# fzaiser/genfer

Measured on AMD Instinct MI355X. Metric: TaylorPoly mul f64 GMAC/s, higher is better.
Workload: dtype f64

## Files before the change

genfer_amd/csrc/gft_api.hip:

```cpp
#include <hip/hip_runtime.h>
#include <dlfcn.h>
#include <rccl/rccl.h>

#include <algorithm>
#include <chrono>
#include <atomic>
#include <cmath>
#include <cstdio>
#include <cstring>
#include <deque>
#include <exception>
#include <functional>
#include <initializer_list>
#include <map>
#include <memory>
#include <tuple>
#include <stdexcept>
#include <string>
#include <vector>

#include "../../include/gftaylor.h"
#include "gft_kernels.hpp"
#include "gft_small_alloc.hpp"
#include "gft_host.hpp"
// ... 159 lines not shown
    size_t peak_total = 0;
    unsigned* d_flag = nullptr;
    double* d_scratch = nullptr;
    unsigned* d_wit = nullptr;
    double* h_pinned = nullptr;
    double* h_mail = nullptr;
    double* d_mail = nullptr;
    unsigned long long mail_seq = 0;
    hipEvent_t events[64] = {};
    static constexpr int IO_EVENTS = 16;
    hipEvent_t io_events[IO_EVENTS] = {};
    int io_next = 0;
    int series_force = 0;
    int series_last = 0;
    int conv_mode = 0;
    static constexpr int pairs_first = 1;
    double pairs_first_max = 1.0e7, pairs_first_max_rank2 = 2.0e8;
    double tiled_min_macs = 2.0e5;
    double tiled_min_override = -1;
    static constexpr double recur_tiled_min_macs = 1.0e300;
    size_t stats[8] = {0, 0, 0, 0, 0, 0, 0, 0};
    size_t stats_ex[4] = {0, 0, 0, 0};
    bool defer = true;
    size_t horner_loop_max = (size_t)1 << 40;
    static constexpr bool fuse_horner = true;
    bool div_wavefront = true;
    bool exp_right = true;
    size_t shallow_max_terms = 256;
    size_t stats_shallow[2] = {0, 0};
    unsigned nf_epoch = 0;
    int conv_variant = -1;
    void* conv_ws = nullptr;
    size_t conv_ws_bytes = 0;
    void ensure_conv_ws(size_t need) {
        if (need <= conv_ws_bytes) return;
        size_t want = std::max<size_t>(std::max(need, std::min<size_t>(2 * conv_ws_bytes, (size_t)1 << 32)), (size_t)8 << 20);
        if (conv_ws) HIP_OK(hipFree(conv_ws));
        conv_ws = nullptr;
        conv_ws_bytes = 0;
        if (hipMalloc(&conv_ws, want) != hipSuccess) {
            (void)hipGetLastError();
            want = need;
            HIP_OK(hipMalloc(&conv_ws, want));
        }
        conv_ws_bytes = want;
    }
    unsigned* next_nf_epoch() {
        if (++nf_epoch == 0) {
            HIP_OK(hipMemsetD32Async((hipDeviceptr_t)(d_flag + 2), 0, 1, stream));
            nf_epoch = 1;
        }
        return d_flag + 2;
    }
    static constexpr size_t HOST_MAX_ELEMS_DEFAULT = 2048;
    static constexpr double HOST_MAX_MACS_DEFAULT = 65536;
    size_t host_max_elems = HOST_MAX_ELEMS_DEFAULT;
    double host_max_macs = HOST_MAX_MACS_DEFAULT;
    std::map<size_t, std::vector<void*>> host_blocks;
};
Runtime& R = *new Runtime;

static size_t size_class(size_t bytes) {
    if (bytes < 256) return 256;
    if (bytes <= (1u << 20)) {
        size_t c = 256;
        while (c < bytes) c <<= 1;
        return c;
    }
    const size_t g = 2u << 20;
// ... 1020 lines not shown
        HIP_OK(hipEventSynchronize(R.events[b]));
        float ms = 0;
        HIP_OK(hipEventElapsedTime(&ms, R.events[a], R.events[b]));
        return ms;
    } catch (const std::exception& e) {
        g_err = e.what();
        return -1.0f;
    }
}
int gft_set_option(const char* name, double value) {
    std::string n = name ? name : "";
    if (n == "horner_loop_max") R.horner_loop_max = value < 0 ? 0 : (size_t)value;
    else if (n == "div_wavefront") R.div_wavefront = value != 0;
    else if (n == "exp_right") R.exp_right = value != 0;
    else if (n == "recur_overlap") R.recur_overlap = value != 0;
    else if (n == "defer") R.defer = value != 0;
    else if (n == "lazy_observe") R.lazy_observe = value != 0;
    else if (n == "batch_dag") R.batch_dag = value != 0;
    else if (n == "lazy_horner") R.lazy_horner = value != 0;
    else if (n == "nz_proofs") R.nz_proofs = value != 0;
    else if (n == "lazy_sum") R.lazy_sum = value != 0;
    else if (n == "async_launch") lq_configure(R.device, value != 0);
    else if (n == "trace_lq_report") lq_report();
    else if (n == "shallow_max_terms") R.shallow_max_terms = value < 0 ? 256 : (size_t)value;
    else if (n == "debug_fail_next_launch") g_fail_next_launch.store(value != 0 ? 1 : 0);
    else if (n == "tiled_min_macs") R.tiled_min_macs = value;
    else if (n == "conv_rb_min_macs") staged_set_rb_min_macs(value);
    else if (n == "conv_rb_pairs") staged_set_rb_pairs(value);
    else if (n == "conv_rb_pairs_cap") staged_set_rb_pairs_cap(value);
    else if (n == "conv_rb_pairs_lanes") staged_set_rb_pairs_lanes(value);
    else if (n == "shallow_pair_min") shallow_set_pair_min(value == -1.0 ? 4096.0 : value);
    else if (n == "tiled_tile") tiled_set_lane_tile((int)value);
    else if (n == "tiled_peel") tiled_set_peel((int)value);
    else if (n == "host_max_elems") R.host_max_elems = value < 0 ? Runtime::HOST_MAX_ELEMS_DEFAULT : (size_t)value;
    else if (n == "host_max_macs") R.host_max_macs = value < 0 ? Runtime::HOST_MAX_MACS_DEFAULT : value;
    else if (n == "series_form") R.series_force = (value == 1 || value == 2) ? (int)value : 0;
    else if (n == "dist_min_macs") dist_set_min_macs(value);
    else if (n == "dist_event_slot") dist_set_event_slot(value);
    else return -1;
    return 0;
}
int gft_set_conv_variant(int v) {
    R.conv_variant = v;
    return 0;
}
int gft_set_conv_mode(int mode) {
    if (mode < 0 || mode > 3) return -1;
    R.conv_mode = mode;
    return 0;
}

int gft_conv_raw(const double* x, const size_t* xshape, const double* y, const size_t* yshape, double* res,
                 const size_t* rshape, size_t ndim, size_t slab_lo, size_t slab_hi, int accumulate) {
    return guard_int([&] {
        typedef Ops<EF64> O;
        O::HV xv{const_cast<double*>(x), 0, dims(xshape, ndim)};
        O::HV yv{const_cast<double*>(y), 0, dims(yshape, ndim)};
        O::HV zv{res, 0, dims(rshape, ndim)};
        for (size_t i = 0; i < ndim; ++i)
            if (xshape[i] > rshape[i] || yshape[i] > rshape[i] || xshape[i] == 0 || yshape[i] == 0)
                throw Error("conv_raw: operand shapes must be non-empty and not exceed the result shape");
        if (ndim > 0 && (slab_lo > slab_hi || slab_hi > rshape[0])) throw Error("conv_raw: bad slab range");
        O::conv(xv, yv, zv, slab_lo, slab_hi, accumulate != 0, false, 0, 0, 0);
        launch_drain();
        return 0;
    });
// ... 564 lines not shown
```

genfer_amd/csrc/gft_conv_tiled.hip:

```cpp
#include <algorithm>
#include <cstdlib>
#include <cstring>
#include <map>
#include <vector>

#include "gft_kernels.hpp"

namespace gft {

namespace {

struct TileSeg {
    unsigned u, a, b;
    unsigned step_begin, step_end;
    int dest;
};

struct RedTile {
    unsigned u, a, b;
    unsigned first, count;
    unsigned slot0;
};

struct TiledArgs {
    unsigned xU, x0, x1, xI;
    unsigned yU, y0, y1, yI;
    unsigned zU, z0, z1, zI;
    unsigned nx8, ny8;
    unsigned nxc, nyc, nb;
    unsigned P1;
    unsigned tsh;
    unsigned slab_axis;
    unsigned slab_lo, slab_hi;
    int accumulate;
    unsigned xcd_remap;
    unsigned cut;
    unsigned lim1;
    size_t zsU, zs0, zs1, zoff;
    const double* xp;
    const double* yp;
    double* z;
    double* ws;
    const TileSeg* segs;
    const unsigned* wg_begin;
    const RedTile* red;
    const unsigned* red_slots;
    const unsigned* guard;
    unsigned guard_epoch;
    unsigned char blk1[8], blk2[8];
};

typedef const double __attribute__((address_space(4))) * cptr_t;

#ifndef GFT_TILED_DEFAULT_VARIANT
#define GFT_TILED_DEFAULT_VARIANT 7
#endif
#ifndef GFT_TILED_PEEL_DEFAULT
#define GFT_TILED_PEEL_DEFAULT -1
#endif
constexpr unsigned PEEL_MIN_EXTENT = 112, PEEL_MIN_INNER = 64;

__device__ inline void loadx(double (&dst)[8], cptr_t p) {
#pragma unroll
    for (int i = 0; i < 8; ++i) dst[i] = p[i];
}

__device__ inline void load8(double (&dst)[8], const double* p) {
#pragma unroll
    for (int i = 0; i < 8; ++i) dst[i] = p[i];
}

__device__ inline void load8_b128(double (&dst)[8], const double* p) {
    const double2* q = reinterpret_cast<const double2*>(__builtin_assume_aligned(p, 16));
#pragma unroll
    for (int i = 0; i < 4; ++i) {
        double2 v = q[i];
        dst[2 * i] = v.x;
        dst[2 * i + 1] = v.y;
    }
}

__device__ inline void fma_rows(double (&acc)[8], const double (&xq)[8], const double (&cur)[8],
                                const double (&prev)[8], int s_lo, int s_hi) {
#pragma unroll
    for (int s = 0; s < 8; ++s) {
        if (s < s_lo || s >= s_hi) continue;
        const double xs = xq[s];
#pragma unroll
        for (int r = 0; r < 8; ++r) {
            const double yv = (r - s >= 0) ? cur[(r - s) & 7] : prev[(8 + r - s) & 7];
            acc[r] = __builtin_fma(xs, yv, acc[r]);
        }
    }
// ... 129 lines not shown
    __builtin_amdgcn_sched_barrier(0);
    if (tri) fma_tri(acc, X1, C);
    unsigned q = q_lo;
    GFT_CHUNK_LOOP(q_hi);
}

struct TileGeom {
    unsigned julo, n_ju, j0lo, n_j0, j1lo, n_j1;
};

__host__ __device__ inline TileGeom tile_geom(const TiledArgs& A, unsigned tsh, unsigned u, unsigned a, unsigned b) {
    TileGeom g;
    const unsigned T0 = 64u >> tsh, T1 = 1u << tsh;
    g.julo = (u + 1 > A.yU) ? (u + 1 - A.yU) : 0;
    unsigned juhi = (u + 1 < A.xU) ? (u + 1) : A.xU;
    g.n_ju = juhi > g.julo ? juhi - g.julo : 0;
    unsigned k0max = (T0 * a + T0 - 1 < A.z0 - 1) ? T0 * a + T0 - 1 : A.z0 - 1;
    g.j0lo = (T0 * a + 1 > A.y0) ? (T0 * a + 1 - A.y0) : 0;
    unsigned j0hi = (k0max + 1 < A.x0) ? (k0max + 1) : A.x0;
    if ((A.cut & 1u) && T0 * a + 1 < j0hi) j0hi = T0 * a + 1;
    g.n_j0 = j0hi > g.j0lo ? j0hi - g.j0lo : 0;
    unsigned k1max = (T1 * b + T1 - 1 < A.z1 - 1) ? T1 * b + T1 - 1 : A.z1 - 1;
    g.j1lo = (T1 * b + 1 > A.y1) ? (T1 * b + 1 - A.y1) : 0;
    unsigned j1hi = (k1max + 1 < A.x1) ? (k1max + 1) : A.x1;
    if ((A.cut & 2u) && T1 * b + 1 < j1hi) j1hi = T1 * b + 1;
    g.n_j1 = j1hi > g.j1lo ? j1hi - g.j1lo : 0;
    return g;
}

constexpr unsigned YPAD = 8;


template <int NW, int VAR, int TSH>
__global__ void __launch_bounds__(NW * 64, 4)
k_conv_tiled(TiledArgs A) {
    constexpr bool FAST = (VAR & 1) != 0;
    constexpr bool NO_WINDOW = (VAR & 64) != 0;
    constexpr bool PEEL = (VAR & 128) != 0;
    extern __shared__ double lds[];
    if (A.guard && *A.guard == A.guard_epoch) return;
    const unsigned tid = threadIdx.x;
    const unsigned lane = tid & 63u;
    const unsigned wave = __builtin_amdgcn_readfirstlane(tid >> 6);
    const unsigned tsh = TSH ? (unsigned)TSH : A.tsh, T1m = (1u << tsh) - 1u, T0 = 64u >> tsh;
    const unsigned l0 = lane >> tsh, l1 = lane & T1m;
    constexpr unsigned NT = NW * 64;

    const unsigned c1 = A.blk1[wave];
    const unsigned c2 = A.blk2[wave];
    const bool has1 = c1 != 0xffu;
    const bool has2 = c2 != 0xffu;

    const unsigned half_row = A.ny8 >> 1;
    const unsigned hr_magic = (1u << 24) / half_row + 1u;
    const size_t y_row_stride = A.ny8;
    const unsigned pf_s0 = (tid * hr_magic) >> 24, pf_col = tid - pf_s0 * half_row;
    const bool pf_mine = pf_s0 < T0;
    double* const lds_lane = lds + (size_t)(l0 << tsh) * A.P1 + YPAD;
    double* const lds_pf = lds + (size_t)(pf_s0 << tsh) * A.P1 + YPAD + 2 * pf_col;

    unsigned wg = blockIdx.x;
    if (A.xcd_remap) wg = (blockIdx.x & 7u) * (gridDim.x >> 3) + (blockIdx.x >> 3);
    const unsigned seg_begin = A.wg_begin[wg], seg_end = A.wg_begin[wg + 1];
    for (unsigned si = seg_begin; si < seg_end; ++si) {
        const TileSeg seg = A.segs[si];
        const unsigned u = seg.u, a = seg.a, b = seg.b;
        const TileGeom g = tile_geom(A, tsh, u, a, b);
        const unsigned k0 = T0 * a + l0, k1 = (b << tsh) + l1;
        bool lane_in = k0 < A.z0 && k1 < A.z1;
        if (A.slab_axis == 1) lane_in = lane_in && k0 >= A.slab_lo && k0 < A.slab_hi;
        else if (A.slab_axis == 2) lane_in = lane_in && k1 >= A.slab_lo && k1 < A.slab_hi;
        unsigned y1lim = A.y1;
        if (PEEL && A.lim1 && (k1 & ~7u) + 1u < y1lim) y1lim = (k1 & ~7u) + 1u;

        double acc1[8], acc2[8];
#pragma unroll
        for (int i = 0; i < 8; ++i) acc1[i] = acc2[i] = 0.0;

        unsigned tj1 = seg.step_begin % g.n_j1;
        unsigned t = seg.step_begin / g.n_j1;
        unsigned tj0 = t % g.n_j0;
        unsigned ju = g.julo + t / g.n_j0, j0 = g.j0lo + tj0, j1 = g.j1lo + tj1;
        unsigned steps_left = seg.step_end - seg.step_begin;
        const unsigned j1_end = g.j1lo + g.n_j1;

        while (steps_left) {
            const unsigned row_steps = steps_left < j1_end - j1 ? steps_left : j1_end - j1;
            const double* ybase = A.yp + (size_t)(u - ju) * A.y0 * A.y1 * y_row_stride;
            if (!NO_WINDOW) {
                __syncthreads();
                for (unsigned p = tid; p < 64 * half_row; p += NT) {
                    unsigned row = (p * hr_magic) >> 24, col = p - row * half_row;
                    unsigned s0 = row >> tsh, s1 = row & T1m;
                    int R0 = (int)(T0 * a + s0) - (int)j0;
                    int R1 = (int)((b << tsh) + s1) - (int)j1;
// ... 63 lines not shown
                double* zrow = A.z + (((size_t)u * A.z0 + k0) * A.z1 + k1) * A.zI;
                if constexpr (PEEL) zrow = A.z + A.zoff + (size_t)u * A.zsU + (size_t)k0 * A.zs0 + (size_t)k1 * A.zs1;
                if (has1) {
#pragma unroll
                    for (int r = 0; r < 8; ++r) {
                        unsigned k2 = 8 * c1 + r;
                        if (k2 < A.zI) zrow[k2] = A.accumulate ? zrow[k2] + acc1[r] : acc1[r];
                    }
                }
                if (has2) {
#pragma unroll
                    for (int r = 0; r < 8; ++r) {
                        unsigned k2 = 8 * c2 + r;
                        if (k2 < A.zI) zrow[k2] = A.accumulate ? zrow[k2] + acc2[r] : acc2[r];
                    }
                }
            }
        } else {
            double* w = A.ws + (size_t)seg.dest * A.nb * 512;
            if (has1) {
                double* d = w + ((size_t)c1 * 64 + lane) * 8;
#pragma unroll
                for (int r = 0; r < 8; ++r) d[r] = acc1[r];
            }
            if (has2) {
                double* d = w + ((size_t)c2 * 64 + lane) * 8;
#pragma unroll
                for (int r = 0; r < 8; ++r) d[r] = acc2[r];
            }
        }
    }
}

__global__ void __launch_bounds__(256) k_conv_reduce(TiledArgs A, unsigned n_red) {
    const unsigned ti = blockIdx.x, c = blockIdx.y;
    if (ti >= n_red) return;
    if (A.guard && *A.guard == A.guard_epoch) return;
    __shared__ double part[3][64][8];
    const RedTile rt = A.red[ti];
    const unsigned lane = threadIdx.x & 63u, q = threadIdx.x >> 6;
    const unsigned k0 = (64u >> A.tsh) * rt.a + (lane >> A.tsh), k1 = (rt.b << A.tsh) + (lane & ((1u << A.tsh) - 1u));
    bool lane_in = k0 < A.z0 && k1 < A.z1;
    if (A.slab_axis == 1) lane_in = lane_in && k0 >= A.slab_lo && k0 < A.slab_hi;
    else if (A.slab_axis == 2) lane_in = lane_in && k1 >= A.slab_lo && k1 < A.slab_hi;
    double v[8];
#pragma unroll
    for (int r = 0; r < 8; ++r) v[r] = 0.0;
    double* zrow = A.z + A.zoff + (size_t)rt.u * A.zsU + (size_t)k0 * A.zs0 + (size_t)k1 * A.zs1;
    if (lane_in) {
        if (q == 0 && A.accumulate) {
#pragma unroll
            for (int r = 0; r < 8; ++r) {
                unsigned k2 = 8 * c + r;
                if (k2 < A.zI) v[r] = zrow[k2];
            }
        }
        const unsigned lo = (unsigned)((unsigned long long)rt.count * q / 4), hi = (unsigned)((unsigned long long)rt.count * (q + 1) / 4);
        unsigned p = lo;
        if (!A.red_slots) {
            const size_t stride = (size_t)A.nb * 512;
            const double* w = A.ws + (size_t)(rt.slot0 + lo) * stride + ((size_t)c * 64 + lane) * 8;
            for (; p + 4 <= hi; p += 4, w += 4 * stride) {
                double t[4][8];
#pragma unroll
                for (int u = 0; u < 4; ++u)
#pragma unroll
                    for (int r = 0; r < 8; ++r) t[u][r] = w[(size_t)u * stride + r];
#pragma unroll
                for (int u = 0; u < 4; ++u)
#pragma unroll
                    for (int r = 0; r < 8; ++r) v[r] += t[u][r];
            }
        }
        for (; p < hi; ++p) {
            const unsigned slot = A.red_slots ? A.red_slots[rt.first + p] : rt.slot0 + p;
            const double* w = A.ws + (size_t)slot * A.nb * 512 + ((size_t)c * 64 + lane) * 8;
#pragma unroll
            for (int r = 0; r < 8; ++r) v[r] += w[r];
        }
        if (q > 0) {
#pragma unroll
            for (int r = 0; r < 8; ++r) part[q - 1][lane][r] = v[r];
        }
    }
    __syncthreads();
    if (q == 0 && lane_in) {
#pragma unroll
        for (int g = 0; g < 3; ++g)
#pragma unroll
            for (int r = 0; r < 8; ++r) v[r] += part[g][lane][r];
#pragma unroll
        for (int r = 0; r < 8; ++r) {
            unsigned k2 = 8 * c + r;
            if (k2 < A.zI) zrow[k2] = v[r];
        }
    }
}

__global__ void __launch_bounds__(256) k_prep_operands(const double* __restrict__ x, double* __restrict__ xp, size_t x_rows,
                                                       unsigned xlen, unsigned nx8, const double* __restrict__ y,
                                                       double* __restrict__ yp, size_t y_rows, unsigned ylen, unsigned ny8,
                                                       unsigned* flag, unsigned epoch) {
    const size_t tx = x_rows * nx8, ty = yp ? y_rows * ny8 : y_rows * ylen;
    bool bad = false;
    for (size_t i = blockIdx.x * (size_t)blockDim.x + threadIdx.x; i < tx + ty; i += (size_t)gridDim.x * blockDim.x) {
        double v;
        if (i < tx) {
            size_t row = i / nx8;
            unsigned col = (unsigned)(i - row * nx8);
            v = col < xlen ? x[row * xlen + col] : 0.0;
            xp[i] = v;
        } else if (yp) {
            size_t k = i - tx, row = k / ny8;
            unsigned col = (unsigned)(k - row * ny8);
            v = col < ylen ? y[row * ylen + col] : 0.0;
            yp[k] = v;
        } else {
            v = y[i - tx];
        }
        if (!((v - v) == 0.0)) bad = true;
    }
    if (__any(bad) && (threadIdx.x & 63) == 0) atomicMax(flag, epoch);
}
// ... 126 lines not shown
    return c;
}

unsigned long long& plan_generation() {
    static unsigned long long g = 0;
    return g;
}

void reset_plan_cache(hipStream_t st) {
    (void)hipStreamSynchronize(st);
    for (auto& kv : plan_cache())
        if (kv.second.d_tables) (void)hipFree(kv.second.d_tables);
    plan_cache().clear();
    plan_generation()++;
    arena().head = 0;
}

int num_cus() {
    static int n = 0;
    if (!n) {
        int dev = 0;
        (void)hipGetDevice(&dev);
        hipDeviceProp_t p;
        if (hipGetDeviceProperties(&p, dev) == hipSuccess) n = p.multiProcessorCount;
        if (n <= 0) n = 256;
    }
    return n;
}

struct PeelSpec {
    unsigned role = 0;
    unsigned cut = 0, lim1 = 0;
    size_t zsU = 0, zs0 = 0, zs1 = 0, zoff = 0;
};

int& tiled_force_tsh() {
    static int v = 0;
    return v;
}

unsigned pick_lane_tile(const TiledArgs& T) {
    auto axis_eff = [](unsigned T, unsigned nx, unsigned ny, unsigned nz) {
        double useful = 0, issued = 0;
        for (unsigned t = 0; t * T < nz; ++t) {
            const unsigned kmax = std::min(T * t + T - 1, nz - 1);
            const unsigned jlo = T * t + 1 > ny ? T * t + 1 - ny : 0, jhi = std::min(kmax + 1, nx);
            if (jhi > jlo) issued += (double)(jhi - jlo) * T;
            for (unsigned k = T * t; k <= kmax; ++k) {
                const unsigned lo = k + 1 > ny ? k + 1 - ny : 0, hi = std::min(k + 1, nx);
                if (hi > lo) useful += hi - lo;
            }
        }
        return issued > 0 ? useful / issued : 0.0;
    };
    const int force = tiled_force_tsh();
    if (force >= 3 && force <= 6) return (unsigned)force;
    double best = -1.0;
    unsigned best_tsh = 3;
    for (unsigned tsh = 3; tsh <= 6; ++tsh) {
        const double e = axis_eff(64u >> tsh, T.x0, T.y0, T.z0) * axis_eff(1u << tsh, T.x1, T.y1, T.z1);
        if (e > best * 1.02) {
            best = e;
            best_tsh = tsh;
        }
    }
    return best_tsh;
// ... 63 lines not shown
    if (a.j0_min != 0 || a.j0_excl != 0 || a.j0_desc != 0) return false;
    T.nx8 = (T.xI + 7) / 8 * 8;
    T.ny8 = (T.yI + 7) / 8 * 8;
    T.nxc = T.nx8 / 8;
    T.nyc = T.ny8 / 8;
    T.nb = (T.zI + 7) / 8;
    T.P1 = V.b128 ? T.ny8 + YPAD + 2 : T.ny8 + YPAD + 1;
    T.tsh = pick_lane_tile(T);
    T.cut = ps.cut;
    T.lim1 = ps.lim1;
    if (ps.role >= 2) {
        T.zsU = ps.zsU; T.zs0 = ps.zs0; T.zs1 = ps.zs1; T.zoff = ps.zoff;
    } else {
        T.zsU = (size_t)T.z0 * T.z1 * T.zI; T.zs0 = (size_t)T.z1 * T.zI; T.zs1 = T.zI; T.zoff = 0;
    }
    T.slab_lo = a.slab_lo;
    T.slab_hi = a.slab_hi;
    T.accumulate = a.accumulate;
    unsigned npairs = (T.nb + 1) / 2;
    P.NW = npairs <= 1 ? 1 : (npairs <= 2 ? 2 : (npairs <= 4 ? 4 : 8));
    P.lds_bytes = (size_t)64 * T.P1 * sizeof(double);
    assign_blocks(T, P.NW);
    return true;
}

struct PlanTables {
    std::vector<TileSeg> segs;
    std::vector<unsigned> wg_begin;
    std::vector<RedTile> red;
    std::vector<unsigned> red_slots;
    bool slots_consecutive = true;
};

bool cut_ranges(Plan& P, PlanTables& tb) {
    const TiledArgs& T = P.base;
    const unsigned TT0 = 64u >> T.tsh, TT1 = 1u << T.tsh;
    struct TileInfo { unsigned u, a, b; unsigned long long steps; };
    std::vector<TileInfo> tiles;
    unsigned u_lo = 0, u_hi = T.zU, a_lo = 0, a_hi = (T.z0 + TT0 - 1) / TT0, b_lo = 0, b_hi = (T.z1 + TT1 - 1) / TT1;
    if (T.slab_axis == 0) {
        u_lo = T.slab_lo;
        u_hi = T.slab_hi;
    } else if (T.slab_axis == 1) {
        a_lo = T.slab_lo / TT0;
        a_hi = (T.slab_hi + TT0 - 1) / TT0;
    } else {
        b_lo = T.slab_lo / TT1;
        b_hi = (T.slab_hi + TT1 - 1) / TT1;
    }
    unsigned long long S = 0;
    for (unsigned u = u_lo; u < u_hi; ++u)
        for (unsigned aa = a_lo; aa < a_hi; ++aa)
            for (unsigned bb = b_lo; bb < b_hi; ++bb) {
                TileGeom g = tile_geom(T, T.tsh, u, aa, bb);
                unsigned long long st = (unsigned long long)g.n_ju * g.n_j0 * g.n_j1;
                if (st == 0 || st > 0xffffffffull) return false;
                tiles.push_back({u, aa, bb, st});
                S += st;
            }
    if (tiles.empty()) return false;
    unsigned wg_per_cu = std::min<unsigned>(16u / P.NW, (unsigned)(160 * 1024 / P.lds_bytes));
    if (wg_per_cu < 1) wg_per_cu = 1;
    unsigned long long n_wg = (unsigned long long)num_cus() * wg_per_cu;
    const unsigned long long per_slot = S / n_wg;
    const unsigned long long fit = per_slot / 190;
    n_wg *= fit >= 8 ? 8u : (fit >= 4 ? 4u : (fit >= 2 ? 2u : 1u));
    constexpr unsigned long long MIN_UNITS = 64;
    const unsigned long long step_units = (unsigned long long)T.nb * (T.nb + 1) / 2 + 3;
    const unsigned long long min_steps =
        std::max<unsigned long long>(1, (MIN_UNITS + 20ull * T.nb + step_units / 2) / step_units);
    if (n_wg > S / min_steps) n_wg = std::max<unsigned long long>(1, S / min_steps);
    P.n_wg = (unsigned)n_wg;

    tb.wg_begin.assign(P.n_wg + 1, 0);
    std::vector<std::vector<unsigned>> tile_slots(tiles.size());
    std::vector<int> tile_direct(tiles.size(), 0);
    unsigned n_slots = 0;
    size_t ti = 0;
    unsigned long long tile_start = 0;
    for (unsigned w = 0; w < P.n_wg; ++w) {
        unsigned long long lo = S * w / n_wg, hi = S * (w + 1) / n_wg;
        tb.wg_begin[w] = (unsigned)tb.segs.size();
        unsigned long long pos = lo;
        while (pos < hi) {
            while (pos >= tile_start + tiles[ti].steps) {
                tile_start += tiles[ti].steps;
                ti++;
            }
            unsigned long long tend = tile_start + tiles[ti].steps;
            unsigned long long e = hi < tend ? hi : tend;
            TileSeg sg = {tiles[ti].u, tiles[ti].a, tiles[ti].b, (unsigned)(pos - tile_start), (unsigned)(e - tile_start), -1};
            if (sg.step_begin == 0 && sg.step_end == tiles[ti].steps) {
                tile_direct[ti] = 1;
            } else {
                sg.dest = (int)n_slots;
                tile_slots[ti].push_back(n_slots);
                n_slots++;
            }
            tb.segs.push_back(sg);
            pos = e;
        }
    }
    tb.wg_begin[P.n_wg] = (unsigned)tb.segs.size();
    for (size_t i = 0; i < tiles.size(); ++i) {
        if (tile_direct[i] || tile_slots[i].empty()) continue;
        RedTile r = {tiles[i].u, tiles[i].a, tiles[i].b, (unsigned)tb.red_slots.size(), (unsigned)tile_slots[i].size(), tile_slots[i][0]};
        for (size_t q = 0; q < tile_slots[i].size(); ++q)
            if (tile_slots[i][q] != r.slot0 + q) tb.slots_consecutive = false;
        for (unsigned sl : tile_slots[i]) tb.red_slots.push_back(sl);
        tb.red.push_back(r);
    }
    P.n_red = (unsigned)tb.red.size();
    P.n_slots = n_slots;
    return true;
}

bool upload_tables(Plan& P, const PlanTables& tb, hipStream_t st) {
    TiledArgs& T = P.base;
    size_t b_segs = tb.segs.size() * sizeof(TileSeg), b_wg = tb.wg_begin.size() * sizeof(unsigned);
    size_t b_red = tb.red.size() * sizeof(RedTile), b_rs = tb.red_slots.size() * sizeof(unsigned);
    auto al = [](size_t x) { return (x + 255) / 256 * 256; };
    size_t total = al(b_segs) + al(b_wg) + al(b_red) + al(b_rs) + 256;
    TableArena& A = arena();
    char *base = nullptr, *hbase = nullptr;
    if (A.ensure() && total <= A.bytes / 4) {
        if (A.head + total > A.bytes) reset_plan_cache(st);
        base = A.dev + A.head;
        hbase = A.host + A.head;
        A.head += total;
    } else {
        if (hipMalloc(&P.d_tables, total) != hipSuccess) return false;
        base = (char*)P.d_tables;
    }
    size_t off = 0;
    auto put = [&](const void* src, size_t bytes) -> void* {
        void* d = base + off;
        if (bytes) {
            if (hbase) std::memcpy(hbase + off, src, bytes);
            else (void)hipMemcpy(d, src, bytes, hipMemcpyHostToDevice);
        }
        off += al(bytes);
        return d;
    };
    T.segs = (const TileSeg*)put(tb.segs.data(), b_segs);
    T.wg_begin = (const unsigned*)put(tb.wg_begin.data(), b_wg);
    T.red = (const RedTile*)put(tb.red.data(), b_red);
    T.red_slots = (const unsigned*)put(tb.red_slots.data(), b_rs);
    if (tb.slots_consecutive) T.red_slots = nullptr;
    if (hbase && hipMemcpyAsync(base, hbase, off, hipMemcpyHostToDevice, st) != hipSuccess) return false;
    return true;
}

bool build_plan(const ConvArgs& a, const Variant& V, const PeelSpec& ps, Plan& P, hipStream_t st) {
    PlanTables tb;
    return canonicalise(a, V, ps, P) && cut_ranges(P, tb) && upload_tables(P, tb, st);
}

template <int NW, int VAR, int TSH>
void launch_main_t(hipStream_t st, const Plan& P, const TiledArgs& T) {
    static bool attr_set = false;
    if (!attr_set) {
        (void)hipFuncSetAttribute(reinterpret_cast<const void*>(&k_conv_tiled<NW, VAR, TSH>),
                                  hipFuncAttributeMaxDynamicSharedMemorySize, 160 * 1024);
        attr_set = true;
    }
    GFT_LAUNCH((k_conv_tiled<NW, VAR, TSH>), dim3(P.n_wg), dim3(NW * 64), P.lds_bytes, st, T);
}
template <int NW, int VAR>
void launch_main_nw(hipStream_t st, const Plan& P, const TiledArgs& T) {
    if (T.tsh == 3) launch_main_t<NW, VAR, 3>(st, P, T);
    else launch_main_t<NW, VAR, 0>(st, P, T);
}
template <int VAR>
void launch_main(hipStream_t st, const Plan& P, const TiledArgs& T) {
    switch (P.NW) {
        case 1: launch_main_nw<1, VAR>(st, P, T); break;
        case 2: launch_main_nw<2, VAR>(st, P, T); break;
        case 4: launch_main_nw<4, VAR>(st, P, T); break;
        default: launch_main_nw<8, VAR>(st, P, T); break;
    }
}

}

void tiled_pad_rows_f64(hipStream_t st, const double* in, double* out, size_t rows, unsigned len, unsigned P, unsigned B) {
    size_t tot = rows * P * B;
    if (!tot) return;
    GFT_LAUNCH(k_pad_rows, dim3((unsigned)std::min<size_t>((tot + 255) / 256, 4096)), dim3(256), 0, st, in, out, rows,
                       len, P, B);
}
void tiled_fold_rows_f64(hipStream_t st, const double* zt, double* z, size_t rows, size_t row_lo, size_t row_hi, unsigned Pz,
                         unsigned B, unsigned zI, int accumulate, const unsigned* guard, unsigned epoch) {
    size_t tot = (row_hi - row_lo) * zI;
    if (!tot) return;
    GFT_LAUNCH(k_fold_rows, dim3((unsigned)std::min<size_t>((tot + 255) / 256, 4096)), dim3(256), 0, st, zt, z, rows,
                       row_lo, row_hi, Pz, B, zI, accumulate, guard, epoch);
}

void tiled_set_lane_tile(int tsh) { tiled_force_tsh() = tsh; }

namespace {

int& tiled_peel_mode() {
    static int v = GFT_TILED_PEEL_DEFAULT;
    return v;
}

const Plan* cached_plan(const ConvArgs& a, const Variant& V, const PeelSpec& ps, hipStream_t st) {
    PlanKey key;
    std::memset(&key, 0, sizeof(key));
    if (a.nd < 2 || a.nd > 4) return nullptr;
    key.v[0] = (unsigned)a.nd | ((unsigned)a.slab_axis << 8) | ((unsigned)tiled_force_tsh() << 16);
    for (int i = 0; i < a.nd; ++i) {
        key.v[1 + i] = a.xs[i];
        key.v[5 + i] = a.ys[i];
        key.v[9 + i] = a.zs[i];
    }
    key.v[13] = a.slab_lo;
    key.v[14] = a.slab_hi;
    key.v[15] = (unsigned)a.accumulate;
    key.v[16] = (unsigned)(a.j0_min | (a.j0_excl << 8) | (a.j0_desc << 16));
    key.v[17] = V.b128;
    key.v[18] = ps.role | (ps.cut << 4) | (ps.lim1 << 8);
    auto& cache = plan_cache();
    auto it = cache.find(key);
    if (it == cache.end()) {
        Plan P;
        if (cache.size() >= 1024) reset_plan_cache(st);
        if (!build_plan(a, V, ps, P, st)) return nullptr;
        it = cache.emplace(key, P).first;
    }
    return &it->second;
}

bool launch_plan(hipStream_t st, const Plan& P, TiledArgs T, const Variant& V) {
    T.xcd_remap = (V.xcd && P.n_wg % 8 == 0) ? 1u : 0u;
    switch (pick_var(V, P.NW)) {
        case 131: launch_main<131>(st, P, T); break;
        case 11: launch_main<11>(st, P, T); break;
        case 3: launch_main<3>(st, P, T); break;
        case 0: launch_main<0>(st, P, T); break;
        case 1: launch_main_nw<8, 1>(st, P, T); break;
#ifdef GFT_TILED_DIAG
        case 17: launch_main_nw<8, 17>(st, P, T); break;
        case 33: launch_main_nw<8, 33>(st, P, T); break;
        case 49: launch_main_nw<8, 49>(st, P, T); break;
        case 65: launch_main_nw<8, 65>(st, P, T); break;
        case 113: launch_main_nw<8, 113>(st, P, T); break;
#endif
        default: return false;
    }
    if (P.n_red) {
        GFT_LAUNCH(k_conv_reduce, dim3(P.n_red, T.nb), dim3(256), 0, st, T, P.n_red);
    }
    return true;
}

struct Operands {
    bool inplace, pack_y;
    size_t o_xp, o_yp, end;
};
Operands operand_layout(const TiledArgs& B, size_t n_slots, const double* x, const double* y, int operands_slack) {
    auto al = [](size_t v) { return (v + 255) / 256 * 256; };
    const size_t x_rows = (size_t)B.xU * B.x0 * B.x1, y_rows = (size_t)B.yU * B.y0 * B.y1;
    Operands o;
    o.inplace = operands_slack && B.nx8 == B.xI && B.ny8 == B.yI && B.nxc >= B.nb && B.nyc >= B.nb && !((uintptr_t)y & 15) &&
                !((uintptr_t)x & 7);
    o.pack_y = !o.inplace && (B.ny8 != B.yI || ((uintptr_t)y & 15));
    o.o_xp = al(n_slots * B.nb * 512 * sizeof(double));
    o.o_yp = o.o_xp + al((x_rows * B.nx8 + 8) * sizeof(double));
    o.end = o.o_yp + al(y_rows * B.ny8 * sizeof(double));
    return o;
}
void bind_operands(hipStream_t st, const Operands& o, const double* x, const double* y, char* wb, unsigned* nf_flag,
                   unsigned nf_epoch, TiledArgs& T) {
    T.ws = (double*)wb;
    if (o.inplace) {
        T.xp = x;
        T.yp = y;
        T.guard = nullptr;
        T.guard_epoch = 0;
        return;
    }
    const size_t x_rows = (size_t)T.xU * T.x0 * T.x1, y_rows = (size_t)T.yU * T.y0 * T.y1;
    double *xp = (double*)(wb + o.o_xp), *yp = (double*)(wb + o.o_yp);
    const size_t tot = x_rows * T.nx8 + (o.pack_y ? y_rows * T.ny8 : y_rows * T.yI);
    GFT_LAUNCH(k_prep_operands, dim3((unsigned)std::min<size_t>((tot + 255) / 256, 2048)), dim3(256), 0, st, x, xp, x_rows, T.xI,
               T.nx8, y, o.pack_y ? yp : nullptr, y_rows, T.yI, T.ny8, nf_flag, nf_epoch);
    T.xp = xp;
    T.yp = o.pack_y ? yp : y;
    T.guard = nf_flag;
    T.guard_epoch = nf_epoch;
}

bool peel_applies(const ConvArgs& a, const Variant& V) {
    const int mode = tiled_peel_mode();
    if (mode == 0) return false;
    if (a.nd != 3 || a.slab_axis != 0 || a.slab_lo != 0 || a.slab_hi != a.zs[0]) return false;
    if (a.j0_min || a.j0_excl || a.j0_desc) return false;
    for (int i = 0; i < 3; ++i)
        if (a.xs[i] != a.zs[i] || a.ys[i] != a.zs[i]) return false;
    const unsigned n0 = a.zs[0], n1 = a.zs[1];
    if (n0 % 8 || n1 % 8 || n0 < 16 || n1 < 16 || a.zs[2] > 128) return false;
    if (!V.fast || !V.b128 || V.compact || V.peel || V.other) return false;
    TiledArgs T;
    std::memset(&T, 0, sizeof(T));
    T.x0 = T.y0 = T.z0 = n0;
    T.x1 = T.y1 = T.z1 = n1;
    if (pick_lane_tile(T) != 3) return false;
    return mode == 1 || (n0 >= PEEL_MIN_EXTENT && n1 >= PEEL_MIN_EXTENT && a.zs[2] >= PEEL_MIN_INNER);
}

int conv_tiled_peel(hipStream_t st, const double* x, const double* y, double* z, const ConvArgs& a, const Variant& V, void* ws,
                    size_t ws_bytes, size_t* ws_needed, unsigned* nf_flag, unsigned nf_epoch, bool* guarded) {
    const unsigned n0 = a.zs[0], n1 = a.zs[1], nI = a.zs[2];
    ConvArgs l0, l1;
    std::memset(&l0, 0, sizeof(l0));
    l0.nd = 4;
    l0.slab_lo = 0;
    l0.slab_hi = 7;
    l0.accumulate = 1;
    l1 = l0;
    Variant VL = V;
    VL.peel = true;
    const unsigned s0x[4] = {7, 1, n1, nI}, s0y[4] = {7, n0 / 8, n1, nI}, s1x[4] = {7, 1, n0, nI}, s1y[4] = {7, n1 / 8, n0, nI};
    for (int i = 0; i < 4; ++i) {
        l0.xs[i] = s0x[i]; l0.ys[i] = l0.zs[i] = s0y[i];
        l1.xs[i] = s1x[i]; l1.ys[i] = l1.zs[i] = s1y[i];
    }
    PeelSpec pm, p0, p1;
    pm.role = 1; pm.cut = 3;
    p0.role = 2; p0.zsU = (size_t)n1 * nI; p0.zs0 = 8 * p0.zsU; p0.zs1 = nI; p0.zoff = p0.zsU;
    p1.role = 3; p1.lim1 = 1; p1.zsU = nI; p1.zs0 = 8 * (size_t)nI; p1.zs1 = (size_t)n1 * nI; p1.zoff = nI;
    Plan PM, P0, P1;
    for (int attempt = 0;; ++attempt) {
        const unsigned long long gen = plan_generation();
        const Plan* q = cached_plan(a, V, pm, st);
        if (!q) return -1;
        PM = *q;
        if (!(q = cached_plan(l0, VL, p0, st))) return -1;
        P0 = *q;
        if (!(q = cached_plan(l1, VL, p1, st))) return -1;
        P1 = *q;
        if (gen == plan_generation()) break;
        if (attempt) return -1;
    }
    const TiledArgs& B = PM.base;
    if (B.tsh != 3) return -1;
    const size_t n8 = B.nx8;
    const Operands o = operand_layout(B, std::max(PM.n_slots, std::max(P0.n_slots, P1.n_slots)), x, y, a.operands_slack);
    const size_t e_w0 = (size_t)7 * (n0 / 8) * n1 * n8, e_s1 = (size_t)7 * n0 * n8, e_w1 = (size_t)7 * (n1 / 8) * n0 * n8;
    auto al = [](size_t v) { return (v + 255) / 256 * 256; };
    const size_t o_w0 = o.end, o_s1 = o_w0 + al(e_w0 * sizeof(double)), o_w1 = o_s1 + al((e_s1 + 8) * sizeof(double)),
                 need = o_w1 + al(e_w1 * sizeof(double)) + 256;
    if (ws && ws_bytes < need) return -1;
    if (ws_needed) *ws_needed = need;
    if (guarded) *guarded = !o.inplace;
    if (!ws) return 1;

    char* wb = (char*)ws;
    double *w0 = (double*)(wb + o_w0), *s1 = (double*)(wb + o_s1), *w1 = (double*)(wb + o_w1);
    TiledArgs T = B;
    bind_operands(st, o, x, y, wb, nf_flag, nf_epoch, T);
    {
        const size_t tot = e_w0 + e_s1 + e_w1;
        GFT_LAUNCH(k_pack_peel, dim3((unsigned)std::min<size_t>((tot + 255) / 256, 4096)), dim3(256), 0, st, x, y, w0, s1, w1, n0, n1,
                   nI, (unsigned)n8);
    }
    T.z = z;
    if (!launch_plan(st, PM, T, V)) return 0;
    TiledArgs T0 = P0.base, T1 = P1.base;
    T0.ws = T1.ws = T.ws;
    T0.z = T1.z = z;
    T0.guard = T1.guard = T.guard;
    T0.guard_epoch = T1.guard_epoch = T.guard_epoch;
    T0.xp = T.yp;
    T0.yp = w0;
    T1.xp = s1;
    T1.yp = w1;
    return launch_plan(st, P0, T0, VL) && launch_plan(st, P1, T1, VL) ? 1 : 0;
}

}

void tiled_set_peel(int mode) { tiled_peel_mode() = mode < 0 ? -1 : (mode ? 1 : 0); }

bool conv_tiled_f64(hipStream_t st, const double* x, const double* y, double* z, const ConvArgs& a, void* ws, size_t ws_bytes,
                    size_t* ws_needed, unsigned* nf_flag, unsigned nf_epoch, bool* guarded, bool* peeled) {
    bool compact_operands = false;
    if (a.nd >= 2 && a.nd <= 4) {
        const unsigned nb = (a.zs[a.nd - 1] + 7) / 8;
        compact_operands = (a.xs[a.nd - 1] + 7) / 8 < nb || (a.ys[a.nd - 1] + 7) / 8 < nb;
    }
    const Variant V = decode_variant(a.variant, compact_operands);
    if (peeled) *peeled = false;
    if (peel_applies(a, V)) {
        const int r = conv_tiled_peel(st, x, y, z, a, V, ws, ws_bytes, ws_needed, nf_flag, nf_epoch, guarded);
        if (r >= 0) {
            if (peeled) *peeled = r == 1;
            return r == 1;
        }
    }
    const Plan* P = cached_plan(a, V, PeelSpec(), st);
    if (!P) return false;
    const Operands o = operand_layout(P->base, P->n_slots, x, y, a.operands_slack);
    const size_t need = o.end + 256;
    if (guarded) *guarded = !o.inplace;
    if (ws_needed) *ws_needed = need;
    if (!ws) return true;
    if (ws_bytes < need) return false;
    TiledArgs T = P->base;
    bind_operands(st, o, x, y, (char*)ws, nf_flag, nf_epoch, T);
    T.z = z;
    return launch_plan(st, *P, T, V);
}

}
```

genfer_amd/csrc/gft_kernels.hpp:

```cpp
#pragma once
#include <hip/hip_runtime.h>

#include <cstddef>
#include <cstdint>
#include <vector>

#include "gft_elem.hpp"
#include "gft_launch.hpp"
#include "gft_wavefront_plan.hpp"

namespace gft {

constexpr int MAXD = 12;

struct Shape {
    int nd;
    unsigned d[MAXD];
};

struct DView {
    double* p;
    size_t plane;
    Shape sh;
};
// ... 276 lines not shown
    static void factor_table(hipStream_t st, int op, unsigned n, unsigned len, const double* m, size_t m_plane,
                             double* tab, size_t tab_plane);
    static void sum_axis(hipStream_t st, const double* in, size_t in_plane, unsigned outer, unsigned len,
                         unsigned inner, size_t axis_stride_outer, double* out, size_t out_plane, int mode);
    static void any_zero(hipStream_t st, const double* p, size_t plane, size_t n, unsigned* state, const Mailbox& mb);
    static void zero_pattern(hipStream_t st, const double* p, size_t plane, const Shape& sh, size_t n, unsigned* state, const Mailbox& mb);
    static void count_neq(hipStream_t st, const double* a, size_t a_plane, const double* b, size_t b_plane,
                          size_t n, unsigned* count);
    static void conv_naive(hipStream_t st, const double* x, size_t x_plane, const double* y, size_t y_plane,
                           double* z, size_t z_plane, const ConvArgs& a);
    static bool conv_shallow(hipStream_t st, const double* x, size_t x_plane, const double* y, size_t y_plane, double* out,
                             size_t out_plane, const ConvArgs& a, const ConvEpi& e);
    static bool conv_line(hipStream_t st, const double* x, size_t x_plane, const double* y, size_t y_plane, double* z, size_t z_plane,
                          const ConvArgs& a);
};

enum SumMode { SUM_SEQ = 0, SUM_UNROLL8 = 1, SUM_WAVE = 2 };

bool conv_tiled_f64(hipStream_t st, const double* x, const double* y, double* z, const ConvArgs& a, void* ws,
                    size_t ws_bytes, size_t* ws_needed, unsigned* nf_flag, unsigned nf_epoch, bool* guarded = nullptr,
                    bool* peeled = nullptr);

template <class E>
bool conv_pairs(hipStream_t st, const double* x, size_t xp, const double* y, size_t yp, double* z, size_t zp, const ConvArgs& a, double max_macs);
void staged_set_rb_min_macs(double v);
void staged_set_rb_pairs(double v);
void staged_set_rb_pairs_cap(double bytes);
void shallow_set_pair_min(double v);
void staged_set_rb_pairs_lanes(double v);
size_t staged_scratch_bytes();
void staged_release_scratch();
void dwf_release_orders();
void tiled_set_lane_tile(int tsh);
void tiled_set_peel(int mode);
void tiled_pad_rows_f64(hipStream_t st, const double* in, double* out, size_t rows, unsigned len, unsigned P, unsigned B);
void tiled_fold_rows_f64(hipStream_t st, const double* zt, double* z, size_t rows, size_t row_lo, size_t row_hi, unsigned Pz,
                         unsigned B, unsigned zI, int accumulate, const unsigned* guard, unsigned epoch);

template <class E>
bool conv_staged(hipStream_t st, const double* x, size_t x_plane, const double* y, size_t y_plane, double* z,
                 size_t z_plane, const ConvArgs& a, bool force);

}
```

Baseline: 29810.

## Merge peeled main and leftover tiled-convolution launches into one kernel with fused reduce

The peeled tiled convolution used to launch the main plan and two leftover plans as separate kernels, each with its own reduction. They are now combined into one kernel that dispatches workgroups by block index, and one reduce kernel that also folds in the leftover partial sums. Each plan gets its own workspace slab. The peel threshold is lowered so more shapes take the peeled path, and an optional exact-fit workspace mode is added. The aim is to cut launch count and serialization between the peel passes, at the cost of a larger workspace and more complex reduction indexing.

```diff
diff --git a/genfer_amd/csrc/gft_api.hip b/genfer_amd/csrc/gft_api.hip
--- a/genfer_amd/csrc/gft_api.hip
+++ b/genfer_amd/csrc/gft_api.hip
@@ -215,9 +215,11 @@
     int conv_variant = -1;
     void* conv_ws = nullptr;
     size_t conv_ws_bytes = 0;
+    bool conv_ws_fit = false;
     void ensure_conv_ws(size_t need) {
-        if (need <= conv_ws_bytes) return;
+        if (conv_ws_fit ? need == conv_ws_bytes : need <= conv_ws_bytes) return;
         size_t want = std::max<size_t>(std::max(need, std::min<size_t>(2 * conv_ws_bytes, (size_t)1 << 32)), (size_t)8 << 20);
+        if (conv_ws_fit) want = need;
         if (conv_ws) HIP_OK(hipFree(conv_ws));
         conv_ws = nullptr;
         conv_ws_bytes = 0;
@@ -1304,6 +1306,13 @@
     else if (n == "shallow_pair_min") shallow_set_pair_min(value == -1.0 ? 4096.0 : value);
     else if (n == "tiled_tile") tiled_set_lane_tile((int)value);
     else if (n == "tiled_peel") tiled_set_peel((int)value);
+    else if (n == "conv_ws_fit") {
+        R.conv_ws_fit = value != 0;
+        if (R.conv_ws) (void)hipFree(R.conv_ws);
+        R.conv_ws = nullptr;
+        R.conv_ws_bytes = 0;
+    }
+    else if (n == "tiled_peel_merge") tiled_set_peel_merge((int)value);
     else if (n == "host_max_elems") R.host_max_elems = value < 0 ? Runtime::HOST_MAX_ELEMS_DEFAULT : (size_t)value;
     else if (n == "host_max_macs") R.host_max_macs = value < 0 ? Runtime::HOST_MAX_MACS_DEFAULT : value;
     else if (n == "series_form") R.series_force = (value == 1 || value == 2) ? (int)value : 0;
diff --git a/genfer_amd/csrc/gft_conv_tiled.hip b/genfer_amd/csrc/gft_conv_tiled.hip
--- a/genfer_amd/csrc/gft_conv_tiled.hip
+++ b/genfer_amd/csrc/gft_conv_tiled.hip
@@ -20,6 +20,7 @@
     unsigned u, a, b;
     unsigned first, count;
     unsigned slot0;
+    unsigned direct;
 };
 
 struct TiledArgs {
@@ -58,7 +59,10 @@
 #ifndef GFT_TILED_PEEL_DEFAULT
 #define GFT_TILED_PEEL_DEFAULT -1
 #endif
-constexpr unsigned PEEL_MIN_EXTENT = 112, PEEL_MIN_INNER = 64;
+#ifndef GFT_TILED_PEEL_RANGES
+#define GFT_TILED_PEEL_RANGES 1
+#endif
+constexpr unsigned PEEL_MIN_EXTENT = 80, PEEL_MIN_INNER = 64;
 
 __device__ inline void loadx(double (&dst)[8], cptr_t p) {
 #pragma unroll
@@ -254,8 +258,7 @@
 
 
 template <int NW, int VAR, int TSH>
-__global__ void __launch_bounds__(NW * 64, 4)
-k_conv_tiled(TiledArgs A) {
+__device__ __forceinline__ void conv_tiled_body(const TiledArgs& A, const unsigned bid, const unsigned nwg) {
     constexpr bool FAST = (VAR & 1) != 0;
     constexpr bool NO_WINDOW = (VAR & 64) != 0;
     constexpr bool PEEL = (VAR & 128) != 0;
@@ -281,8 +284,8 @@
     double* const lds_lane = lds + (size_t)(l0 << tsh) * A.P1 + YPAD;
     double* const lds_pf = lds + (size_t)(pf_s0 << tsh) * A.P1 + YPAD + 2 * pf_col;
 
-    unsigned wg = blockIdx.x;
-    if (A.xcd_remap) wg = (blockIdx.x & 7u) * (gridDim.x >> 3) + (blockIdx.x >> 3);
+    unsigned wg = bid;
+    if (A.xcd_remap) wg = (bid & 7u) * (nwg >> 3) + (bid >> 3);
     const unsigned seg_begin = A.wg_begin[wg], seg_end = A.wg_begin[wg + 1];
     for (unsigned si = seg_begin; si < seg_end; ++si) {
         const TileSeg seg = A.segs[si];
@@ -412,6 +415,34 @@
     }
 }
 
+template <int NW, int VAR, int TSH>
+__global__ void __launch_bounds__(NW * 64, 4)
+k_conv_tiled(TiledArgs A) {
+    conv_tiled_body<NW, VAR, TSH>(A, blockIdx.x, gridDim.x);
+}
+
+struct PeeledArgs {
+    TiledArgs m, l0, l1;
+    unsigned nM, nMp, n0, n0p, n1;
+};
+template <int NW, int LT>
+__global__ void __launch_bounds__(NW * 64, 4) k_conv_tiled_peeled(PeeledArgs K) {
+    unsigned b = blockIdx.x;
+    if (b < K.nMp) {
+        if (b < K.nM) conv_tiled_body<NW, 3, 3>(K.m, b, K.nM);
+        return;
+    }
+    b -= K.nMp;
+    const TiledArgs* L = &K.l0;
+    unsigned n = K.n0;
+    if (b >= K.n0p) {
+        b -= K.n0p;
+        L = &K.l1;
+        n = K.n1;
+    }
+    if (b < n) conv_tiled_body<NW, 131, LT>(*L, b, n);
+}
+
 __global__ void __launch_bounds__(256) k_conv_reduce(TiledArgs A, unsigned n_red) {
     const unsigned ti = blockIdx.x, c = blockIdx.y;
     if (ti >= n_red) return;
@@ -469,6 +500,96 @@
         for (int g = 0; g < 3; ++g)
 #pragma unroll
             for (int r = 0; r < 8; ++r) v[r] += part[g][lane][r];
+#pragma unroll
+        for (int r = 0; r < 8; ++r) {
+            unsigned k2 = 8 * c + r;
+            if (k2 < A.zI) zrow[k2] = v[r];
+        }
+    }
+}
+
+__device__ inline void add_leftover(double (&v)[8], const TiledArgs& L, unsigned m, unsigned kc0, unsigned kc1, unsigned c) {
+    const unsigned tsh = L.tsh, T0 = 64u >> tsh, T1m = (1u << tsh) - 1u;
+    const unsigned na = (L.z0 + T0 - 1u) / T0, nbt = (L.z1 + T1m) >> tsh;
+    const unsigned lane = ((kc0 & (T0 - 1u)) << tsh) | (kc1 & T1m);
+    const RedTile rt = L.red[((size_t)m * na + (kc0 >> (6u - tsh))) * nbt + (kc1 >> tsh)];
+    const size_t stride = (size_t)L.nb * 512;
+    const double* w = L.ws + (size_t)rt.slot0 * stride + ((size_t)c * 64 + lane) * 8;
+    if (rt.direct) {
+#pragma unroll
+        for (int r = 0; r < 8; ++r) v[r] += w[r];
+        return;
+    }
+    for (unsigned q = 0; q < 4; ++q) {
+        const unsigned lo = (unsigned)((unsigned long long)rt.count * q / 4), hi = (unsigned)((unsigned long long)rt.count * (q + 1) / 4);
+        double t[8];
+#pragma unroll
+        for (int r = 0; r < 8; ++r) t[r] = q ? 0.0 : v[r];
+        for (unsigned p = lo; p < hi; ++p)
+#pragma unroll
+            for (int r = 0; r < 8; ++r) t[r] += w[(size_t)p * stride + r];
+#pragma unroll
+        for (int r = 0; r < 8; ++r) v[r] = q ? v[r] + t[r] : t[r];
+    }
+}
+
+__global__ void __launch_bounds__(256) k_conv_reduce_peeled(PeeledArgs K, unsigned n_tiles) {
+    const TiledArgs& A = K.m;
+    const unsigned ti = blockIdx.x, c = blockIdx.y;
+    if (ti >= n_tiles) return;
+    if (A.guard && *A.guard == A.guard_epoch) return;
+    __shared__ double part[3][64][8];
+    const RedTile rt = A.red[ti];
+    const unsigned lane = threadIdx.x & 63u, q = threadIdx.x >> 6;
+    const unsigned k0 = 8u * rt.a + (lane >> 3), k1 = 8u * rt.b + (lane & 7u);
+    const bool lane_in = k0 < A.z0 && k1 < A.z1;
+    double v[8];
+#pragma unroll
+    for (int r = 0; r < 8; ++r) v[r] = 0.0;
+    double* zrow = A.z + (size_t)k0 * A.zs0 + (size_t)k1 * A.zs1;
+    if (lane_in) {
+        if (q == 0 && (A.accumulate || rt.direct)) {
+#pragma unroll
+            for (int r = 0; r < 8; ++r) {
+                unsigned k2 = 8 * c + r;
+                if (k2 < A.zI) v[r] = zrow[k2];
+            }
+        }
+        if (!rt.direct) {
+            const unsigned lo = (unsigned)((unsigned long long)rt.count * q / 4), hi = (unsigned)((unsigned long long)rt.count * (q + 1) / 4);
+            const size_t stride = (size_t)A.nb * 512;
+            const double* w = A.ws + (size_t)(rt.slot0 + lo) * stride + ((size_t)c * 64 + lane) * 8;
+            unsigned p = lo;
+            for (; p + 4 <= hi; p += 4, w += 4 * stride) {
+                double t[4][8];
+#pragma unroll
+                for (int u = 0; u < 4; ++u)
+#pragma unroll
+                    for (int r = 0; r < 8; ++r) t[u][r] = w[(size_t)u * stride + r];
+#pragma unroll
+                for (int u = 0; u < 4; ++u)
+#pragma unroll
+                    for (int r = 0; r < 8; ++r) v[r] += t[u][r];
+            }
+            for (; p < hi; ++p, w += stride)
+#pragma unroll
+                for (int r = 0; r < 8; ++r) v[r] += w[r];
+            if (q > 0) {
+#pragma unroll
+                for (int r = 0; r < 8; ++r) part[q - 1][lane][r] = v[r];
+            }
+        }
+    }
+    __syncthreads();
+    if (q == 0 && lane_in) {
+        if (!rt.direct) {
+#pragma unroll
+            for (int g = 0; g < 3; ++g)
+#pragma unroll
+                for (int r = 0; r < 8; ++r) v[r] += part[g][lane][r];
+        }
+        if (k0 & 7u) add_leftover(v, K.l0, (k0 & 7u) - 1u, k0 >> 3, k1, c);
+        if (k1 & 7u) add_leftover(v, K.l1, (k1 & 7u) - 1u, k1 >> 3, k0, c);
 #pragma unroll
         for (int r = 0; r < 8; ++r) {
             unsigned k2 = 8 * c + r;
@@ -661,6 +782,8 @@
     unsigned role = 0;
     unsigned cut = 0, lim1 = 0;
     size_t zsU = 0, zs0 = 0, zs1 = 0, zoff = 0;
+    unsigned ranges = 1;
+    unsigned merged = 0;
 };
 
 int& tiled_force_tsh() {
@@ -790,7 +913,7 @@
     bool slots_consecutive = true;
 };
 
-bool cut_ranges(Plan& P, PlanTables& tb) {
+bool cut_ranges(Plan& P, PlanTables& tb, const PeelSpec& ps) {
     const TiledArgs& T = P.base;
     const unsigned TT0 = 64u >> T.tsh, TT1 = 1u << T.tsh;
     struct TileInfo { unsigned u, a, b; unsigned long long steps; };
@@ -822,7 +945,8 @@
     unsigned long long n_wg = (unsigned long long)num_cus() * wg_per_cu;
     const unsigned long long per_slot = S / n_wg;
     const unsigned long long fit = per_slot / 190;
-    n_wg *= fit >= 8 ? 8u : (fit >= 4 ? 4u : (fit >= 2 ? 2u : 1u));
+    if (ps.role >= 2) n_wg *= ps.ranges;
+    else n_wg *= fit >= 8 ? 8u : (fit >= 4 ? 4u : (fit >= 2 ? 2u : 1u));
     constexpr unsigned long long MIN_UNITS = 64;
     const unsigned long long step_units = (unsigned long long)T.nb * (T.nb + 1) / 2 + 3;
     const unsigned long long min_steps =
@@ -848,9 +972,9 @@
             unsigned long long tend = tile_start + tiles[ti].steps;
             unsigned long long e = hi < tend ? hi : tend;
             TileSeg sg = {tiles[ti].u, tiles[ti].a, tiles[ti].b, (unsigned)(pos - tile_start), (unsigned)(e - tile_start), -1};
-            if (sg.step_begin == 0 && sg.step_end == tiles[ti].steps) {
-                tile_direct[ti] = 1;
-            } else {
+            const bool whole = sg.step_begin == 0 && sg.step_end == tiles[ti].steps;
+            if (whole) tile_direct[ti] = 1;
+            if (!whole || (ps.merged && ps.role >= 2)) {
                 sg.dest = (int)n_slots;
                 tile_slots[ti].push_back(n_slots);
                 n_slots++;
@@ -861,8 +985,10 @@
     }
     tb.wg_begin[P.n_wg] = (unsigned)tb.segs.size();
     for (size_t i = 0; i < tiles.size(); ++i) {
-        if (tile_direct[i] || tile_slots[i].empty()) continue;
-        RedTile r = {tiles[i].u, tiles[i].a, tiles[i].b, (unsigned)tb.red_slots.size(), (unsigned)tile_slots[i].size(), tile_slots[i][0]};
+        if (!ps.merged && (tile_direct[i] || tile_slots[i].empty())) continue;
+        RedTile r = {tiles[i].u, tiles[i].a, tiles[i].b, (unsigned)tb.red_slots.size(), (unsigned)tile_slots[i].size(),
+                     tile_slots[i].empty() ? 0u : tile_slots[i][0], (unsigned)tile_direct[i]};
+        if (ps.merged && !tile_direct[i] && tile_slots[i].empty()) return false;
         for (size_t q = 0; q < tile_slots[i].size(); ++q)
             if (tile_slots[i][q] != r.slot0 + q) tb.slots_consecutive = false;
         for (unsigned sl : tile_slots[i]) tb.red_slots.push_back(sl);
@@ -911,7 +1037,7 @@
 
 bool build_plan(const ConvArgs& a, const Variant& V, const PeelSpec& ps, Plan& P, hipStream_t st) {
     PlanTables tb;
-    return canonicalise(a, V, ps, P) && cut_ranges(P, tb) && upload_tables(P, tb, st);
+    return canonicalise(a, V, ps, P) && cut_ranges(P, tb, ps) && (!ps.merged || tb.slots_consecutive) && upload_tables(P, tb, st);
 }
 
 template <int NW, int VAR, int TSH>
@@ -939,6 +1065,31 @@
     }
 }
 
+template <int NW, int LT>
+void launch_peeled_t(hipStream_t st, const PeeledArgs& K, size_t lds_bytes, unsigned n_tiles) {
+    static bool attr_set = false;
+    if (!attr_set) {
+        (void)hipFuncSetAttribute(reinterpret_cast<const void*>(&k_conv_tiled_peeled<NW, LT>),
+                                  hipFuncAttributeMaxDynamicSharedMemorySize, 160 * 1024);
+        attr_set = true;
+    }
+    GFT_LAUNCH((k_conv_tiled_peeled<NW, LT>), dim3(K.nMp + K.n0p + K.n1), dim3(NW * 64), lds_bytes, st, K);
+    GFT_LAUNCH(k_conv_reduce_peeled, dim3(n_tiles, K.m.nb), dim3(256), 0, st, K, n_tiles);
+}
+template <int NW>
+void launch_peeled_nw(hipStream_t st, const PeeledArgs& K, size_t lds_bytes, unsigned n_tiles) {
+    if (K.l0.tsh == 3 && K.l1.tsh == 3) launch_peeled_t<NW, 3>(st, K, lds_bytes, n_tiles);
+    else launch_peeled_t<NW, 0>(st, K, lds_bytes, n_tiles);
+}
+void launch_peeled(hipStream_t st, unsigned NW, const PeeledArgs& K, size_t lds_bytes, unsigned n_tiles) {
+    switch (NW) {
+        case 1: launch_peeled_nw<1>(st, K, lds_bytes, n_tiles); break;
+        case 2: launch_peeled_nw<2>(st, K, lds_bytes, n_tiles); break;
+        case 4: launch_peeled_nw<4>(st, K, lds_bytes, n_tiles); break;
+        default: launch_peeled_nw<8>(st, K, lds_bytes, n_tiles); break;
+    }
+}
+
 }
 
 void tiled_pad_rows_f64(hipStream_t st, const double* in, double* out, size_t rows, unsigned len, unsigned P, unsigned B) {
@@ -958,6 +1109,11 @@
 void tiled_set_lane_tile(int tsh) { tiled_force_tsh() = tsh; }
 
 namespace {
+
+int& tiled_peel_merge() {
+    static int v = 1;
+    return v;
+}
 
 int& tiled_peel_mode() {
     static int v = GFT_TILED_PEEL_DEFAULT;
@@ -979,7 +1135,7 @@
     key.v[15] = (unsigned)a.accumulate;
     key.v[16] = (unsigned)(a.j0_min | (a.j0_excl << 8) | (a.j0_desc << 16));
     key.v[17] = V.b128;
-    key.v[18] = ps.role | (ps.cut << 4) | (ps.lim1 << 8);
+    key.v[18] = ps.role | (ps.cut << 4) | (ps.lim1 << 8) | (ps.merged << 12) | (ps.ranges << 16);
     auto& cache = plan_cache();
     auto it = cache.find(key);
     if (it == cache.end()) {
@@ -1014,18 +1170,19 @@
     return true;
 }
 
+size_t slab_bytes(const Plan& P) { return (size_t)P.n_slots * P.base.nb * 512 * sizeof(double); }
 struct Operands {
     bool inplace, pack_y;
     size_t o_xp, o_yp, end;
 };
-Operands operand_layout(const TiledArgs& B, size_t n_slots, const double* x, const double* y, int operands_slack) {
+Operands operand_layout(const TiledArgs& B, size_t slabs, const double* x, const double* y, int operands_slack) {
     auto al = [](size_t v) { return (v + 255) / 256 * 256; };
     const size_t x_rows = (size_t)B.xU * B.x0 * B.x1, y_rows = (size_t)B.yU * B.y0 * B.y1;
     Operands o;
     o.inplace = operands_slack && B.nx8 == B.xI && B.ny8 == B.yI && B.nxc >= B.nb && B.nyc >= B.nb && !((uintptr_t)y & 15) &&
                 !((uintptr_t)x & 7);
     o.pack_y = !o.inplace && (B.ny8 != B.yI || ((uintptr_t)y & 15));
-    o.o_xp = al(n_slots * B.nb * 512 * sizeof(double));
+    o.o_xp = al(slabs);
     o.o_yp = o.o_xp + al((x_rows * B.nx8 + 8) * sizeof(double));
     o.end = o.o_yp + al(y_rows * B.ny8 * sizeof(double));
     return o;
@@ -1086,7 +1243,10 @@
         l0.xs[i] = s0x[i]; l0.ys[i] = l0.zs[i] = s0y[i];
         l1.xs[i] = s1x[i]; l1.ys[i] = l1.zs[i] = s1y[i];
     }
+    const bool merge = tiled_peel_merge() != 0;
     PeelSpec pm, p0, p1;
+    pm.merged = p0.merged = p1.merged = merge ? 1u : 0u;
+    p0.ranges = p1.ranges = GFT_TILED_PEEL_RANGES;
     pm.role = 1; pm.cut = 3;
     p0.role = 2; p0.zsU = (size_t)n1 * nI; p0.zs0 = 8 * p0.zsU; p0.zs1 = nI; p0.zoff = p0.zsU;
     p1.role = 3; p1.lim1 = 1; p1.zsU = nI; p1.zs0 = 8 * (size_t)nI; p1.zs1 = (size_t)n1 * nI; p1.zoff = nI;
@@ -1105,10 +1265,13 @@
     }
     const TiledArgs& B = PM.base;
     if (B.tsh != 3) return -1;
+    if (merge && (P0.NW != PM.NW || P1.NW != PM.NW)) return -1;
     const size_t n8 = B.nx8;
-    const Operands o = operand_layout(B, std::max(PM.n_slots, std::max(P0.n_slots, P1.n_slots)), x, y, a.operands_slack);
+    auto al = [](size_t v) { return (v + 255) / 256 * 256; };
+    const size_t o_l0 = merge ? al(slab_bytes(PM)) : 0, o_l1 = merge ? o_l0 + al(slab_bytes(P0)) : 0;
+    const size_t slabs = merge ? o_l1 + al(slab_bytes(P1)) : std::max(slab_bytes(PM), std::max(slab_bytes(P0), slab_bytes(P1)));
+    const Operands o = operand_layout(B, slabs, x, y, a.operands_slack);
     const size_t e_w0 = (size_t)7 * (n0 / 8) * n1 * n8, e_s1 = (size_t)7 * n0 * n8, e_w1 = (size_t)7 * (n1 / 8) * n0 * n8;
-    auto al = [](size_t v) { return (v + 255) / 256 * 256; };
     const size_t o_w0 = o.end, o_s1 = o_w0 + al(e_w0 * sizeof(double)), o_w1 = o_s1 + al((e_s1 + 8) * sizeof(double)),
                  need = o_w1 + al(e_w1 * sizeof(double)) + 256;
     if (ws && ws_bytes < need) return -1;
@@ -1126,9 +1289,10 @@
                    nI, (unsigned)n8);
     }
     T.z = z;
-    if (!launch_plan(st, PM, T, V)) return 0;
+    if (!merge && !launch_plan(st, PM, T, V)) return 0;
     TiledArgs T0 = P0.base, T1 = P1.base;
-    T0.ws = T1.ws = T.ws;
+    T0.ws = (double*)(wb + o_l0);
+    T1.ws = (double*)(wb + o_l1);
     T0.z = T1.z = z;
     T0.guard = T1.guard = T.guard;
     T0.guard_epoch = T1.guard_epoch = T.guard_epoch;
@@ -1136,12 +1300,23 @@
     T0.yp = w0;
     T1.xp = s1;
     T1.yp = w1;
-    return launch_plan(st, P0, T0, VL) && launch_plan(st, P1, T1, VL) ? 1 : 0;
+    if (!merge) return launch_plan(st, P0, T0, VL) && launch_plan(st, P1, T1, VL) ? 1 : 0;
+    PeeledArgs K;
+    K.m = T; K.l0 = T0; K.l1 = T1;
+    K.nM = PM.n_wg; K.n0 = P0.n_wg; K.n1 = P1.n_wg;
+    K.nMp = (K.nM + 7u) & ~7u;
+    K.n0p = (K.n0 + 7u) & ~7u;
+    K.m.xcd_remap = (V.xcd && K.nM % 8 == 0) ? 1u : 0u;
+    K.l0.xcd_remap = (V.xcd && K.n0 % 8 == 0) ? 1u : 0u;
+    K.l1.xcd_remap = (V.xcd && K.n1 % 8 == 0) ? 1u : 0u;
+    launch_peeled(st, PM.NW, K, std::max(PM.lds_bytes, std::max(P0.lds_bytes, P1.lds_bytes)), PM.n_red);
+    return 1;
 }
 
 }
 
 void tiled_set_peel(int mode) { tiled_peel_mode() = mode < 0 ? -1 : (mode ? 1 : 0); }
+void tiled_set_peel_merge(int on) { tiled_peel_merge() = on ? 1 : 0; }
 
 bool conv_tiled_f64(hipStream_t st, const double* x, const double* y, double* z, const ConvArgs& a, void* ws, size_t ws_bytes,
                     size_t* ws_needed, unsigned* nf_flag, unsigned nf_epoch, bool* guarded, bool* peeled) {
@@ -1161,7 +1336,7 @@
     }
     const Plan* P = cached_plan(a, V, PeelSpec(), st);
     if (!P) return false;
-    const Operands o = operand_layout(P->base, P->n_slots, x, y, a.operands_slack);
+    const Operands o = operand_layout(P->base, slab_bytes(*P), x, y, a.operands_slack);
     const size_t need = o.end + 256;
     if (guarded) *guarded = !o.inplace;
     if (ws_needed) *ws_needed = need;
diff --git a/genfer_amd/csrc/gft_kernels.hpp b/genfer_amd/csrc/gft_kernels.hpp
--- a/genfer_amd/csrc/gft_kernels.hpp
+++ b/genfer_amd/csrc/gft_kernels.hpp
@@ -332,6 +332,7 @@
 void staged_release_scratch();
 void dwf_release_orders();
 void tiled_set_lane_tile(int tsh);
+void tiled_set_peel_merge(int on);
 void tiled_set_peel(int mode);
 void tiled_pad_rows_f64(hipStream_t st, const double* in, double* out, size_t rows, unsigned len, unsigned P, unsigned B);
 void tiled_fold_rows_f64(hipStream_t st, const double* zt, double* z, size_t rows, size_t row_lo, size_t row_hi, unsigned Pz,
```

After: 29920 (median of 3 runs). No clear change (+0.4%).
